# paullric/tempestmodel

Hardware: AMD Instinct MI355X
Metric: element-DOF-updates/s (JW baroclinic wave ne30 np4 L30, ARS343 IMEX) (higher is better)
Workload: dtype f64

## Files before the change

include/tempest_mi355x.h:

```cpp
#ifndef TEMPEST_MI355X_H
#define TEMPEST_MI355X_H

#ifdef __cplusplus
extern "C" {
#endif

#define TMX_ABI_VERSION 5

#define TMX_OK                 0
#define TMX_ERR_INVALID       -1
#define TMX_ERR_UNSUPPORTED   -2
#define TMX_ERR_DEVICE        -3
#define TMX_ERR_SINGULAR      -4
#define TMX_ERR_COMM          -5

typedef struct tmx_engine tmx_engine;

enum {
	TMX_OP_INTERP_NODE_TO_REDGE = 0,
	TMX_OP_INTERP_REDGE_TO_NODE,
	TMX_OP_DIFF_NODE_TO_NODE,
	TMX_OP_DIFF_NODE_TO_REDGE,
	TMX_OP_DIFF_REDGE_TO_NODE,
	TMX_OP_DIFF_REDGE_TO_REDGE,
// ... 185 lines not shown
	TMX_INFO_PHYSICS_KERNEL
};
long long tmx_info(tmx_engine * e, int what);

int tmx_set_option(tmx_engine * e, const char * name, double value);
int tmx_get_option(tmx_engine * e, const char * name, double * value);
typedef void (*tmx_dgbsv_fn)(const int * n, const int * kl, const int * ku, const int * nrhs, double * ab, const int * ldab, int * ipiv,
	double * b, const int * ldb, int * info);
int tmx_lu_flavour_from_dgbsv(tmx_engine * e, tmx_dgbsv_fn dgbsv);
int tmx_options_report(tmx_engine * e, char * buf, int cap);
int tmx_options_from_environment(tmx_engine * e);

int tmx_plan_get(tmx_engine * e, int what, int * out, int cap);
int tmx_plan_get_matrices(tmx_engine * e, double * out, int cap);
int tmx_debug_unique_tables(tmx_engine * e, int tile_shape, int what, int * out, int cap);
int tmx_debug_program_unique(int scheme, int first_step, int last_step);
int tmx_debug_program_mixed(int scheme, int first_step, int last_step, int instance);
int tmx_debug_program_rayleigh(int scheme, int first_step, int last_step);
int tmx_debug_program_prefix(int scheme, int first_step, int last_step, int * pairs, int * terms, int cap);
int tmx_debug_walk_segments(int option, int ntiles, int rows, int target_wavefronts);
int tmx_debug_h_timing(tmx_engine * e, unsigned long long * out);
int tmx_debug_h_walk_timing(tmx_engine * e, unsigned long long * out);

int tmx_debug_dss_loopback(tmx_engine ** engines, int n, int instance);
int tmx_debug_loopback_group(tmx_engine ** engines, int n);
int tmx_debug_comm_selftest(tmx_engine * e);

int tmx_debug_pivot_stats(tmx_engine * e, int enable, unsigned long long out[2]);

int tmx_debug_program_copies(int scheme, int mode, int steps, int share, int * copies, int * shared);
// ... 16 lines not shown
```

tempestmodel_amd/csrc/tmx_device.h:

```cpp
#pragma once
#include "tmx_internal.h"
#include "tmx_refmath.h"

#ifndef TMX_H_FUSE_W
#define TMX_H_FUSE_W 1
#endif
#ifndef KT_H
#define KT_H 4
#endif

#ifdef TMX_LU_NOFMA
#define LU_UPD(a, l, u) ((a) - (l) * (u))
#else
#define LU_UPD(a, l, u) __builtin_fma(-(l), (u), (a))
#endif
#ifndef TMX_STORE_PRED
#define TMX_STORE_PRED true
#endif
#ifndef TMX_TAIL
#define TMX_TAIL 2
#endif
#ifndef TMX_SEARCH_TREE
#define TMX_SEARCH_TREE 0
#endif
// ... 443 lines not shown
#endif
	return (base < 0) ? -1 : base + ((lane >> 2) & 3) * nj + (lane & 3);
}

template <bool UQ> __device__ __forceinline__ bool wg_tile(const KParams & p, int nyb, int & tile_ix, int & yb) {
	if (!UQ) { tile_ix = blockIdx.x; yb = blockIdx.y; return true; }
	if (p.u_xcd) return xcd_tile(p.u_ntiles, nyb, tile_ix, yb);
	tile_ix = blockIdx.x % p.u_ntiles; yb = blockIdx.x / p.u_ntiles;
	return yb < nyb;
}
static inline dim3 wg_grid(bool uq, const KParams & p, int ntiles, int nyb) {
	if (!uq) return dim3(ntiles, nyb);
	return dim3(p.u_xcd ? 8 * ((ntiles + 7) / 8) * nyb : ntiles * nyb);
}

template <int NV, int RL>
__device__ __forceinline__ void seam_store(const KParams & p, double (*srow)[RL], int lane_, int sdst, int sred, const double (&v)[NV],
	double * __restrict__ xo, const int (&slab)[NV], int nv)
{
	const int lane = lds_pos<RL != 64>(lane_);
#ifdef TMX_ABL_UQ_DSTORES
	{
		const int c = min((int)(blockIdx.x & 1023) * 64 + lane, p.NSS - 1);
#pragma unroll
		for (int t = 0; t < NV; t++) if (t < nv) xo[(size_t)slab[t] * p.NSS + c] = v[t];
		return;
	}
#endif
#pragma unroll
	for (int t = 0; t < NV; t++) if (t < nv) srow[t][lane] = v[t];
	__builtin_amdgcn_fence(__ATOMIC_RELEASE, "wavefront");
// ... 8 lines not shown
		const int l1 = lds_pos<RL != 64>((sred >> 4) & 63);
#pragma unroll
		for (int t = 0; t < NV; t++) if (t < nv) o[t] = 0.5 * (v[t] + srow[t][l1]);
	} else if (n == 4) {
		const int l1 = lds_pos<RL != 64>((sred >> 4) & 63), l2 = lds_pos<RL != 64>((sred >> 10) & 63), l3 = lds_pos<RL != 64>((sred >> 16) & 63);
#pragma unroll
		for (int t = 0; t < NV; t++) if (t < nv) {
			const double p0 = v[t] + srow[t][l1], p1 = srow[t][l2] + srow[t][l3];
			o[t] = 0.5 * (0.5 * p0 + 0.5 * p1);
		}
	}
	if (sdst >= 0) {
#pragma unroll
		for (int t = 0; t < NV; t++) if (t < nv) xo[(size_t)slab[t] * p.NSS + sdst] = o[t];
	} else {
		const int q = -2 - sdst;
#pragma unroll
		for (int t = 0; t < NV; t++) if (t < nv) p.part[(size_t)slab[t] * p.NP + q] = o[t];
	}
}

__device__ __forceinline__ void lds_barrier() { asm volatile("s_waitcnt lgkmcnt(0)\n\ts_barrier" ::: "memory"); }
template <int NV>
__device__ __forceinline__ void block_seam_store(const KParams & p, double (*xrow)[256], int pos, int sdst, int sred, const double (&v)[NV],
	double * __restrict__ xo, const int (&slab)[NV], unsigned vmask)
{
#pragma unroll
	for (int t = 0; t < NV; t++) if ((vmask >> t) & 1u) xrow[t][pos] = v[t];
	lds_barrier();
	if (sdst == -1) return;
	const int n = sred & 15;
	double o[NV];
#pragma unroll
	for (int t = 0; t < NV; t++) o[t] = v[t];
	if (n == 2) {
		const int l1 = (sred >> 4) & 255;
#pragma unroll
		for (int t = 0; t < NV; t++) if ((vmask >> t) & 1u) o[t] = 0.5 * (v[t] + xrow[t][l1]);
	} else if (n == 4) {
		const int l1 = (sred >> 4) & 255, l2 = (sred >> 12) & 255, l3 = (sred >> 20) & 255;
#pragma unroll
		for (int t = 0; t < NV; t++) if ((vmask >> t) & 1u) {
			const double p0 = v[t] + xrow[t][l1], p1 = xrow[t][l2] + xrow[t][l3];
			o[t] = 0.5 * (0.5 * p0 + 0.5 * p1);
		}
	}
	if (sdst >= 0) {
#pragma unroll
		for (int t = 0; t < NV; t++) if ((vmask >> t) & 1u) xo[(size_t)slab[t] * p.NSS + sdst] = o[t];
	} else {
		const int q = -2 - sdst;
#pragma unroll
		for (int t = 0; t < NV; t++) if ((vmask >> t) & 1u) p.part[(size_t)slab[t] * p.NP + q] = o[t];
	}
}
```

tempestmodel_amd/csrc/tmx_hostshared.h:

```cpp
#pragma once
#include "tmx_internal.h"
#include <pthread.h>
#include <algorithm>
#include <cmath>
#include <cstdarg>
#include <cstdio>
#include <cstring>
#include <dlfcn.h>
#include <map>
#include <mutex>
#include <numeric>
#include <functional>
#include <thread>

static inline bool plan_only(const tmx_engine * e) { return e->cfg.device == -2; }

typedef struct { char internal[128]; } nccl_uid;
typedef int (*fn_ncclGetUniqueId)(nccl_uid *);
typedef int (*fn_ncclCommInitRank)(void **, int, nccl_uid, int);
typedef int (*fn_ncclCommDestroy)(void *);
typedef int (*fn_ncclGroupStart)(void);
typedef int (*fn_ncclGroupEnd)(void);
typedef int (*fn_ncclSend)(const void *, size_t, int, int, void *, hipStream_t);
typedef int (*fn_ncclRecv)(void *, size_t, int, int, void *, hipStream_t);
// ... 33 lines not shown

template <class T> static int dev_upload(T ** d, const std::vector<T> & h, size_t * bytes) {
	const size_t n = h.size() ? h.size() : 1;
	HIPCHK(hipMalloc((void **)d, n * sizeof(T)));
	if (h.size()) HIPCHK(hipMemcpy(*d, h.data(), h.size() * sizeof(T), hipMemcpyHostToDevice));
	*bytes += n * sizeof(T);
	return TMX_OK;
}

static inline int col_of(const PatchInfo & P, int i, int j) {
	const int a = (i - 1) / TMX_NP, ii = (i - 1) % TMX_NP, b = (j - 1) / TMX_NP, jj = (j - 1) % TMX_NP;
	return (P.elem_base + a * P.neb + b) * TMX_NQ + ii * TMX_NP + jj;
}


static inline size_t p2p_header_bytes(int n_ranks) { return (((size_t)2 * n_ranks * sizeof(unsigned long long)) + 255) / 256 * 256; }

KParams make_params(const tmx_engine * e);
int launch_check(const char * what);
int settle_instance(tmx_engine * e, int ix, bool read_only = false);
int check_ready(tmx_engine * e);
int check_inst(tmx_engine * e, int ix, bool read_only = false);
double * inst(tmx_engine * e, int ix);
void interp_orphan(tmx_engine * e);
const double * inst_uv(tmx_engine * e, int ix);
void drop_readers(tmx_engine * e, int x);
double * uinst(tmx_engine * e, int ix);
const double * uinst_uv(tmx_engine * e, int ix);
int u_own_uv(tmx_engine * e, int ix, bool total = false);
void u_written(tmx_engine * e, int x);
// ... 47 lines not shown
```

tempestmodel_amd/csrc/tmx_k_exchange.hip:

```cpp
#include "tmx_device.h"


#ifndef TMX_DSS_LPT
#define TMX_DSS_LPT 1
#endif
#ifndef TMX_DSS_MINWG
#define TMX_DSS_MINWG 5
#endif
__global__ __launch_bounds__(256, TMX_DSS_MINWG) void k_dss(KParams p, double * __restrict__ x, const double * __restrict__ ghost,
	const int * __restrict__ gbase, const int * __restrict__ gstride, int ngroups, const int * __restrict__ gcols,
	const int * __restrict__ gn, const int * __restrict__ gx, const int * __restrict__ gtype, const double * __restrict__ xmat, int nt, int g0)
{
	const int L = p.L;
	const size_t NS = (size_t)p.NS;
	int bx, by;
	if (!xcd_tile((ngroups - g0 + 63) / 64, (L + 1 + 4 * TMX_DSS_LPT - 1) / (4 * TMX_DSS_LPT), bx, by)) return;
	const int g = g0 + bx * 64 + threadIdx.x;
	const int kk0 = (by * 4 + WAVE_UNIFORM(threadIdx.y)) * TMX_DSS_LPT;
	if (g >= ngroups || kk0 > L) return;
	const int n = gn[g];
	const int4 c4 = *(const int4 *)(gcols + g * 4);
	const int c[4] = { c4.x, c4.y, c4.z, c4.w };
	const int xi = gx[g];
	const int gt = gtype[g];
// ... 62 lines not shown
		}
	}
#undef DSS_SCALAR
	}
}

void tmxk_dss(tmx_engine * e, const KParams & p, double * x, int g0, int g1) {
	if (g1 <= g0) return;
	const int nx = (g1 - g0 + 63) / 64, ny = (p.L + 1 + 4 * TMX_DSS_LPT - 1) / (4 * TMX_DSS_LPT);
	dim3 blk(64, 4), grd(8 * ((nx + 7) / 8) * ny);
	hipLaunchKernelGGL(k_dss, grd, blk, 0, e->stream, p, x, (const double *)e->d_ghost, (const int *)e->d_ghost_base,
		(const int *)e->d_ghost_stride, g1,
		(const int *)e->d_grp_cols, (const int *)e->d_grp_n, (const int *)e->d_grp_x, (const int *)e->d_grp_type, (const double *)e->d_xmat, e->nt, g0);
}

__global__ __launch_bounds__(256) void k_pack(int nslab, size_t NS, int nsend,
	const double * __restrict__ x, const int * __restrict__ cols, const int * __restrict__ base,
	const int * __restrict__ stride, double * __restrict__ buf)
{
	const int i = blockIdx.x * 256 + threadIdx.x;
	const int sl = blockIdx.y;
	if (i >= nsend) return;
	buf[(size_t)base[i] + (size_t)sl * stride[i]] = x[(size_t)sl * NS + cols[i]];
}

void tmxk_pack(tmx_engine * e, const KParams & p, const double * x) {
	if (e->nsend == 0) return;
	dim3 blk(256), grd((e->nsend + 255) / 256, e->nslab);
	hipLaunchKernelGGL(k_pack, grd, blk, 0, e->stream, e->nslab, (size_t)p.NS, e->nsend,
		x, (const int *)e->d_send_cols, (const int *)e->d_send_base, (const int *)e->d_send_stride, e->d_sendbuf);
}

__global__ __launch_bounds__(256) void k_pack_p2p(int nslab, size_t NS, int nsend,
	const double * __restrict__ x, const int * __restrict__ cols, const int * __restrict__ within,
	const int * __restrict__ stride, const int * __restrict__ peer, double * const * __restrict__ dst)
{
	const int i = blockIdx.x * 256 + threadIdx.x;
	const int sl = blockIdx.y;
	if (i >= nsend) return;
	dst[peer[i]][(size_t)sl * stride[i] + within[i]] = x[(size_t)sl * NS + cols[i]];
}

__global__ __launch_bounds__(64) void k_p2p_signal_wait(int npeers, const int * __restrict__ peers, unsigned long long * const * __restrict__ flag_dst,
	const unsigned long long * own, unsigned long long seq, int * __restrict__ fail, unsigned long long timeout_ticks)
{
	for (int q = threadIdx.x; q < npeers; q += 64) {
		__threadfence_system();
		__hip_atomic_store(flag_dst[peers[q]], seq, __ATOMIC_RELEASE, __HIP_MEMORY_SCOPE_SYSTEM);
	}
	const bool failed = (__hip_atomic_load(fail, __ATOMIC_RELAXED, __HIP_MEMORY_SCOPE_AGENT) & TMX_FLAG_COMM) != 0;
	for (int q = threadIdx.x; q < npeers && !failed; q += 64) {
		const unsigned long long t0 = wall_clock64();
		while (__hip_atomic_load(own + peers[q], __ATOMIC_ACQUIRE, __HIP_MEMORY_SCOPE_SYSTEM) < seq) {
			__builtin_amdgcn_s_sleep(8);
			if (timeout_ticks && wall_clock64() - t0 > timeout_ticks) { atomicOr(fail, TMX_FLAG_COMM); break; }
		}
	}
	__threadfence_system();
}

void tmxk_pack_p2p(tmx_engine * e, const KParams & p, const double * x, int buf) {
	if (e->nsend == 0) return;
	dim3 blk(256), grd((e->nsend + 255) / 256, e->nslab);
	hipLaunchKernelGGL(k_pack_p2p, grd, blk, 0, e->stream, e->nslab, (size_t)p.NS, e->nsend,
		x, (const int *)e->d_send_cols, (const int *)e->d_send_within, (const int *)e->d_send_stride, (const int *)e->d_send_peer,
		(double * const *)(e->d_p2p_dst + (size_t)buf * e->cfg.n_ranks));
}

void tmxuk_pack(tmx_engine * e) {
	if (e->nsend == 0) return;
	dim3 blk(256), grd((e->nsend + 255) / 256, e->nslab);
	hipLaunchKernelGGL(k_pack, grd, blk, 0, e->stream, e->nslab, (size_t)e->u.NP, e->nsend,
		(const double *)e->u.d_part, (const int *)e->u.d_send_slots, (const int *)e->d_send_base, (const int *)e->d_send_stride, e->d_sendbuf);
}
void tmxuk_pack_p2p(tmx_engine * e, int buf) {
	if (e->nsend == 0) return;
	dim3 blk(256), grd((e->nsend + 255) / 256, e->nslab);
	hipLaunchKernelGGL(k_pack_p2p, grd, blk, 0, e->stream, e->nslab, (size_t)e->u.NP, e->nsend,
		(const double *)e->u.d_part, (const int *)e->u.d_send_slots, (const int *)e->d_send_within, (const int *)e->d_send_stride, (const int *)e->d_send_peer,
		(double * const *)(e->d_p2p_dst + (size_t)buf * e->cfg.n_ranks));
}

void tmxk_p2p_signal_wait(tmx_engine * e, hipStream_t s, int buf, unsigned long long seq) {
	const unsigned long long timeout_ticks = 100000000ull * (unsigned long long)e->p2p_timeout_s;
	hipLaunchKernelGGL(k_p2p_signal_wait, dim3(1), dim3(64), 0, s, e->p2p_npeers, (const int *)e->d_p2p_peers,
		(unsigned long long * const *)(e->d_p2p_flag + (size_t)buf * e->cfg.n_ranks),
		(const unsigned long long *)e->p2p_block + (size_t)buf * e->cfg.n_ranks, seq, e->d_flag, timeout_ticks);
}



__global__ __launch_bounds__(256) void k_lincomb(size_t n, double * __restrict__ dst, LinTerms t) {
	size_t i = (size_t)blockIdx.x * 256 + threadIdx.x;
	const size_t stride = (size_t)gridDim.x * 256;
	for (; i < n; i += stride) {
// ... 202 lines not shown
```

tempestmodel_amd/csrc/tmx_k_horizontal.hip:

```cpp
#include "tmx_device.h"


#ifdef TMX_H_TIMING
#define HT_WAVES 65536
__device__ unsigned long long g_h_rec[8][HT_WAVES][8];
#define HT_DECL long long ht_ = __builtin_readcyclecounter(); long long hts_[7] = { 0, 0, 0, 0, 0, 0, 0 }
#define HT_MARK(i) do { const long long t1_ = __builtin_readcyclecounter(); hts_[i] += t1_ - ht_; ht_ = t1_; } while (0)
#define HT_END(NT_) do { if (threadIdx.x == 0) { const unsigned w_ = ((blockIdx.x * gridDim.y + blockIdx.y) * KT_H + threadIdx.y) % HT_WAVES; \
	for (int q_ = 0; q_ < 7; q_++) g_h_rec[(NT_) & 7][w_][q_] = (unsigned long long)hts_[q_]; g_h_rec[(NT_) & 7][w_][7] = 1ull; } } while (0)
void tmxk_h_timing_read(unsigned long long * out) {
	static std::vector<unsigned long long> h((size_t)8 * HT_WAVES * 8);
	hipMemcpyFromSymbol(h.data(), HIP_SYMBOL(g_h_rec), h.size() * sizeof(unsigned long long));
	for (int i = 0; i < 128; i++) out[i] = 0;
	for (int nt = 0; nt < 8; nt++) for (int w = 0; w < HT_WAVES; w++) if (h[((size_t)nt * HT_WAVES + w) * 8 + 7])
		for (int q = 0; q < 8; q++) out[nt * 8 + q] += h[((size_t)nt * HT_WAVES + w) * 8 + q];
	std::fill(h.begin(), h.end(), 0ull);
	hipMemcpyToSymbol(HIP_SYMBOL(g_h_rec), h.data(), h.size() * sizeof(unsigned long long));
}
#else
#define HT_DECL
#define HT_MARK(i)
#define HT_END(NT_)
void tmxk_h_timing_read(unsigned long long * out) { for (int i = 0; i < 128; i++) out[i] = 0; }
#endif
// ... 301 lines not shown
		}
		outU = bU + tU; outV = bV + tV;
		if (k < 2) { uv01[(size_t)k * NS + col] = outU; uv01[(size_t)(2 + k) * NS + col] = outV; }
		if (k < L - 1) { outU += tUhi; outV += tVhi; }
		if (k > 0) { outU += tUlo; outV += tVlo; }
		outR = bR - tR; outT = bT - tT;
		if (withW) outW = bW + tW;
		if (!UQ) {
			stu(xup + sU, colb, outU); stu(xup + sV, colb, outV); stu(xup + sR, colb, outR); stu(xup + sT, colb, outT);
			if (withW) stu(xup + TMX_SLAB_W(L, k) * NS, colb, outW);
		}
	}
	if (UQ && !MF) {
		const double v[5] = { outU, outV, outR, outT, outW };
		const int slab[5] = { TMX_SLAB_U(L, k), TMX_SLAB_V(L, k), TMX_SLAB_R(L, k), TMX_SLAB_T(L, k), TMX_SLAB_W(L, k) };
		seam_store<5, TMX_UQ_ROWLEN(UQ)>(p, &s[ty][1], lane, sdst, sred, v, xup, slab, (TMX_H_FUSE_W && ty > 0) ? 5 : 4);
	}
#ifdef TMX_H_TIMING
	asm volatile("s_waitcnt vmcnt(0)" ::: "memory");
#endif
	HT_MARK(6);
	HT_END(NT);
}

template <int NT, bool UQ, bool EM, bool DM = false>
__global__ __launch_bounds__(256) void k_h_w_update(KParams p, LinTerms xbase, double * xup,
	const double * __restrict__ ucz, const double * __restrict__ uv01, double dt, int stride, EmitTerms em)
{
	__shared__ double sw[UQ ? 4 : 1][1][64];
	const int L = p.L;
	const size_t NS = (size_t)p.NS;
// ... 462 lines not shown
	el_stiff(s[ty], sSw[ty], ep, { 0, 2, 4 }, { 1, 3, 5 }, { 6, 7 }, ida, idb, wa, wb, ga, gb);

	const double oW = el_scalar_update(bW, dt, 1.0 / je, nu_s, wa[2], wb[2]);
	double oT = 0, oR = 0, oU = 0, oV = 0;
	if (actn) {
		const double invJ = 1.0 / jn;
		oT = el_scalar_update(bT, dt, invJ, nu_s, wa[0], wb[0]);
		oR = el_scalar_update(bR, dt, invJ, nu_s, wa[1], wb[1]);
		const ElPair up = el_vector_update(nu_d, nu_v, j2d, c2a0, c2a1, c2b1, ga[0], gb[0], ga[1], gb[1]);
		oU = bU - dt * up.a;
		oV = bV - dt * up.b;
	}
	if (UQ) {
		const double v[5] = { oW, oT, oR, oU, oV };
		const int slab[5] = { TMX_SLAB_W(L, kk), TMX_SLAB_T(L, kk), TMX_SLAB_R(L, kk), TMX_SLAB_U(L, kk), TMX_SLAB_V(L, kk) };
		if constexpr (BLK) block_seam_store<5>(p, xs, ty * 64 + lane, sdst, sred, v, xout, slab, (kk < L) ? 31u : 1u);
		else seam_store<5, TMX_UQ_ROWLEN(UQ)>(p, &s[ty][0], lane, sdst, sred, v, xout, slab, (kk < L) ? 5 : 1);
		return;
	}
	xout[TMX_SLAB_W(L, kk) * NS + col] = oW;
	if (actn) {
		xout[TMX_SLAB_T(L, kk) * NS + col] = oT;
		xout[TMX_SLAB_R(L, kk) * NS + col] = oR;
		xout[TMX_SLAB_U(L, kk) * NS + col] = oU;
		xout[TMX_SLAB_V(L, kk) * NS + col] = oV;
	}
}

void tmxk_hypervis(tmx_engine * e, const KParams & p, const double * xsrc, const double * xbase, double * xout,
	double dt, double nu_s, double nu_d, double nu_v, int scale, bool pull_dss) {
	const int ntiles = p.quads ? e->launch_tiles : p.NS / 64, nyb = (p.L + 1 + 3) / 4;
	dim3 blk(64, 4);
// ... 349 lines not shown
```

tempestmodel_amd/csrc/tmx_k_hwalk.hip:

```cpp
#include "tmx_device.h"

#ifdef TMX_H_TIMING
#define HW_WAVES 32768
__device__ unsigned long long g_hw_rec[8][HW_WAVES][8];
#define HW_DECL long long hw_ = __builtin_readcyclecounter(); long long hws_[7] = { 0, 0, 0, 0, 0, 0, 0 }
#define HW_MARK(i) do { const long long t1_ = __builtin_readcyclecounter(); hws_[i] += t1_ - hw_; hw_ = t1_; } while (0)
#define HW_END(NT_) do { if (threadIdx.x == 0) { const unsigned w_ = blockIdx.x % HW_WAVES; \
	for (int q_ = 0; q_ < 7; q_++) g_hw_rec[(NT_) & 7][w_][q_] = (unsigned long long)hws_[q_]; g_hw_rec[(NT_) & 7][w_][7] = 1ull; } } while (0)
void tmxk_h_walk_timing_read(unsigned long long * out) {
	static std::vector<unsigned long long> h((size_t)8 * HW_WAVES * 8);
	hipMemcpyFromSymbol(h.data(), HIP_SYMBOL(g_hw_rec), h.size() * sizeof(unsigned long long));
	for (int i = 0; i < 128; i++) out[i] = 0;
	for (int nt = 0; nt < 8; nt++) for (int w = 0; w < HW_WAVES; w++) if (h[((size_t)nt * HW_WAVES + w) * 8 + 7])
		for (int q = 0; q < 8; q++) out[nt * 8 + q] += h[((size_t)nt * HW_WAVES + w) * 8 + q];
	std::fill(h.begin(), h.end(), 0ull);
	hipMemcpyToSymbol(HIP_SYMBOL(g_hw_rec), h.data(), h.size() * sizeof(unsigned long long));
}
#else
#define HW_DECL
#define HW_MARK(i)
#define HW_END(NT_)
void tmxk_h_walk_timing_read(unsigned long long * out) { for (int i = 0; i < 128; i++) out[i] = 0; }
#endif

// ... 410 lines not shown
				double ub0 = 0.0, vb0 = 0.0;
				ub0 += OPK(TMX_OP_INTERP_NODE_TO_REDGE, 0, 0) * uh0; ub0 += OPK(TMX_OP_INTERP_NODE_TO_REDGE, 0, 1) * uh;
				vb0 += OPK(TMX_OP_INTERP_NODE_TO_REDGE, 0, 0) * vh0; vb0 += OPK(TMX_OP_INTERP_NODE_TO_REDGE, 0, 1) * vh;
				double e0, e1, e2, ea, eb_;
				met_eval(mc, etac[L], e0, e1, e2, ea, eb_);
				extra = -(e0 * ub0 + e1 * vb0) / e2; vmask |= 32u;
			}
			if (k == L - 1) {
				double xWl[NX];
				terms_load<NT, PM, DM>(xbase.src, dmask, TMX_SLAB_W(L, L), SS, NSD, cb, gd, xWl);
				extra = lin_reduce<NT, PM>(xbase, xWl); xslab = TMX_SLAB_W(L, L); vmask |= 32u;
				if (EM) stu(em.xp + TMX_SLAB_W(L, L) * SS, cb, emit_value<NT>(em, xWl));
			}
			const double v[6] = { outU, outV, outR, outT, outW, extra };
			const int slab[6] = { TMX_SLAB_U(L, k), TMX_SLAB_V(L, k), TMX_SLAB_R(L, k), TMX_SLAB_T(L, k), TMX_SLAB_W(L, k), xslab };
			block_seam_store<6>(p, xs[k & 1], pos, sdst, sred, v, xup, slab, vmask);
		} else {
			{
				const double v[5] = { outU, outV, outR, outT, outW };
				const int slab[5] = { TMX_SLAB_U(L, k), TMX_SLAB_V(L, k), TMX_SLAB_R(L, k), TMX_SLAB_T(L, k), TMX_SLAB_W(L, k) };
				seam_store<5, RL>(p, &s[0], lane, sdst, sred, v, xup, slab, (k > 0) ? 5 : 4);
			}
			if (k == 0) { uh0 = uh; vh0 = vh; }
			if (k == 1) {
				wave_sync();
				double ub0 = 0.0, vb0 = 0.0;
				ub0 += OPK(TMX_OP_INTERP_NODE_TO_REDGE, 0, 0) * uh0; ub0 += OPK(TMX_OP_INTERP_NODE_TO_REDGE, 0, 1) * uh;
				vb0 += OPK(TMX_OP_INTERP_NODE_TO_REDGE, 0, 0) * vh0; vb0 += OPK(TMX_OP_INTERP_NODE_TO_REDGE, 0, 1) * vh;
				double e0, e1, e2, ea, eb_;
				met_eval(mc, etac[L], e0, e1, e2, ea, eb_);
				const double v1[1] = { -(e0 * ub0 + e1 * vb0) / e2 };
				const int slab1[1] = { TMX_SLAB_W(L, 0) };
				seam_store<1, RL>(p, &s[0], lane, sdst, sred, v1, xup, slab1, 1);
			}
		}
		wave_sync();
// ... 230 lines not shown
		if (actn) {
			oT = c.bT - dt * invJ * nu_s * (uaT + ubT);
			oR = c.bR - dt * invJ * nu_s * (uaR + ubR);
			const double upa = nu_d * dad - nu_v * j2d * (c2a1 * dac + c2b1 * dbc);
			const double upb = nu_d * dbd + nu_v * j2d * (c2a0 * dac + c2a1 * dbc);
			oU = c.bU - dt * upa;
			oV = c.bV - dt * upb;
		}
		wave_sync();
		c = nx;
		asm volatile("" : "+v"(c.W), "+v"(c.T), "+v"(c.R), "+v"(c.U), "+v"(c.V));
		if (HB) asm volatile("" : "+v"(c.bW), "+v"(c.bT), "+v"(c.bR), "+v"(c.bU), "+v"(c.bV));
		{
			const double v[5] = { oW, oT, oR, oU, oV };
			const int slab[5] = { TMX_SLAB_W(L, kk), TMX_SLAB_T(L, kk), TMX_SLAB_R(L, kk), TMX_SLAB_U(L, kk), TMX_SLAB_V(L, kk) };
			seam_store<5, RL>(p, &s[0], lane, here ? sdst : -1, sred, v, xout, slab, actn ? 5 : 1);
		}
		wave_sync();
	};
	Lev C, N;
	load_level(C, k0);
	wave_sync();
	for (int kl = k0; kl < k1; kl++) {
		const int kk = WAVE_UNIFORM(kl);
		level(kk, C, N, N, min(kk + 1, k1 - 1));
	}
}

bool tmxk_hv_walk_ok(const tmx_engine * e, const KParams & p) { return p.t_ucol != nullptr && e->opt_hv_walk != 0 && !tmxu_blocks_on(e, 2); }

void tmxk_hv_walk(tmx_engine * e, const KParams & p, const double * xsrc, const double * xbase, double * xout, double dt, double nu_s, double nu_d, double nu_v, int scale) {
// ... 11 lines not shown
```

tempestmodel_amd/csrc/tmx_plan.hip:

```cpp
#include "tmx_hostshared.h"


struct NodeRef { int patch, i, j; };

struct Nodes {
	const tmx_engine * e;
	std::vector<size_t> poff;
	explicit Nodes(const tmx_engine * e_) : e(e_), poff(e_->cfg.n_patches + 1, 0) {
		for (int p = 0; p < e->cfg.n_patches; p++) poff[p + 1] = poff[p] + (size_t)e->patches[p].na * e->patches[p].nb;
	}
	int id(int p, int i, int j) const { return (int)(poff[p] + (size_t)i * e->patches[p].nb + j); }
	NodeRef ref(int id) const {
		const int p = (int)(std::upper_bound(poff.begin(), poff.end(), (size_t)id) - poff.begin()) - 1;
		const int loc = id - (int)poff[p];
		return NodeRef{ p, loc / e->patches[p].nb, loc % e->patches[p].nb };
	}
	bool local(int id) const { return e->patches[ref(id).patch].owner == e->cfg.rank; }
	int col(int id) const { const NodeRef nr = ref(id); return col_of(e->patches[nr.patch], nr.i, nr.j); }
};
typedef std::vector<std::vector<int>> Groups;

static int uf_find(std::vector<int> & par, int x) {
	while (par[x] != x) { par[x] = par[par[x]]; x = par[x]; }
	return x;
// ... 401 lines not shown
		for (const std::vector<int> * t : { &plan.send_base, &plan.send_stride, &plan.ghost_base, &plan.ghost_stride }) v.insert(v.end(), t->begin(), t->end());
	} else if (what == 10) {
		v = plan.send_cols;
	} else return -1;
	if (out) { if ((int)v.size() > cap) return -1; if (!v.empty()) memcpy(out, v.data(), v.size() * sizeof(int)); }
	return (int)v.size();
}

extern "C" int tmx_plan_get_matrices(tmx_engine * e, double * out, int cap) {
	if (!e || !e->finalized) return -1;
	const PlanHost & plan = e->plan;
	if (out) { if ((int)plan.xmat.size() > cap) return -1; if (!plan.xmat.empty()) memcpy(out, plan.xmat.data(), plan.xmat.size() * sizeof(double)); }
	return (int)plan.xmat.size();
}

extern "C" int tmx_debug_unique_tables(tmx_engine * e, int tile_shape, int what, int * out, int cap) {
	if (!e || !e->finalized || tile_shape < 0 || tile_shape > 4) return -1;
	UniqueLayout keep = e->u;
	e->u = UniqueLayout(); e->u.tile_shape = tile_shape;
	UniqueTables T;
	const int r = tmxu_tables(e, T);
	const UniqueLayout u = e->u;
	e->u = keep;
	if (r) return -1;
	std::vector<int> v;
	switch (what) {
		case 0: v = { u.NU, u.NUS, u.NTS, u.nslots, u.ngroups, u.ngroups_local, u.n_early, u.n_late, u.b_ngroups, u.b_ngroups_local, u.nblocks, u.nb_early, u.nb_late }; break;
		case 13: v = T.b_sdst; break; case 14: v = T.b_sred; break; case 15: v = T.blk_info; break; case 16: v = T.b_gsrc; break; case 17: v = T.b_gdst; break; case 18: v = T.b_gn; break;
		case 19: v = T.blks_early; break; case 20: v = T.blks_late; break;
		case 1: v = T.t_dcol; break; case 2: v = T.t_ucol; break; case 3: v = T.t_sdst; break; case 4: v = T.t_sred; break;
// ... 8 lines not shown
```

tempestmodel_amd/csrc/tmx_unique.hip:

```cpp
#include "tmx_device.h"
#include "tmx_hostshared.h"
#include <algorithm>
#include <cstring>
#include <map>

static int floor_half(int v) { return (v >= 0) ? v / 2 : -((-v + 1) / 2); }
static int sign_of(int v) { return (v > 0) - (v < 0); }
static void gilbert_rec(int x, int y, int ax, int ay, int bx, int by, std::vector<std::pair<int, int>> & out) {
	const int w = std::abs(ax + ay), h = std::abs(bx + by);
	const int dax = sign_of(ax), day = sign_of(ay), dbx = sign_of(bx), dby = sign_of(by);
	if (h == 1) { for (int q = 0; q < w; q++) { out.push_back({ x, y }); x += dax; y += day; } return; }
	if (w == 1) { for (int q = 0; q < h; q++) { out.push_back({ x, y }); x += dbx; y += dby; } return; }
	int ax2 = floor_half(ax), ay2 = floor_half(ay), bx2 = floor_half(bx), by2 = floor_half(by);
	const int w2 = std::abs(ax2 + ay2), h2 = std::abs(bx2 + by2);
	if (2 * w > 3 * h) {
		if ((w2 % 2) && w > 2) { ax2 += dax; ay2 += day; }
		gilbert_rec(x, y, ax2, ay2, bx, by, out);
		gilbert_rec(x + ax2, y + ay2, ax - ax2, ay - ay2, bx, by, out);
	} else {
		if ((h2 % 2) && h > 2) { bx2 += dbx; by2 += dby; }
		gilbert_rec(x, y, bx2, by2, ax2, ay2, out);
		gilbert_rec(x + bx2, y + by2, ax, ay, bx - bx2, by - by2, out);
		gilbert_rec(x + (ax - dax) + (bx2 - dbx), y + (ay - day) + (by2 - dby), -bx2, -by2, -(ax - ax2), -(ay - ay2), out);
	}
// ... 366 lines not shown
	if (u.form[slot] == 2) {
		if (!keep_u) { u.form[slot] = 0; u.n_uform--; }
		return TMX_OK;
	}
	double * xd = e->d_state + (size_t)slot * e->inst_stride;
	const double * xu = u.d_ustate + (size_t)u.uslot[slot] * u.ustride;
	const int ny = std::min(e->nslab, 64);
	hipLaunchKernelGGL(k_u_to_d, dim3((e->ncol + 255) / 256, ny), dim3(256), 0, e->stream, e->nslab, (size_t)e->NS, (size_t)u.NUS, e->ncol, xu, xd, (const int *)u.d_ucol_of_dcol);
	u.conversions++;
	if (keep_u) u.form[slot] = 2;
	else { u.form[slot] = 0; u.n_uform--; }
	return TMX_OK;
}


__global__ __launch_bounds__(256) void k_slots_from_u(int nslab, size_t NUS, size_t NP, int nslots, const double * __restrict__ xu, double * __restrict__ part,
	const int * __restrict__ slot_ucol)
{
	const int q = blockIdx.x * 256 + threadIdx.x;
	if (q >= nslots) return;
	const int uu = slot_ucol[q];
	for (int s = blockIdx.y; s < nslab; s += gridDim.y) part[(size_t)s * NP + q] = xu[(size_t)s * NUS + uu];
}

void tmxuk_slots_from_u(tmx_engine * e, const double * xu) {
	const UniqueLayout & u = e->u;
	if (u.nslots == 0) return;
	hipLaunchKernelGGL(k_slots_from_u, dim3((u.nslots + 255) / 256, std::min(e->nslab, 64)), dim3(256), 0, e->stream, e->nslab, (size_t)u.NUS, (size_t)u.NP, u.nslots, xu,
		u.d_part, (const int *)u.d_slot_ucol);
}

template <int vc>
__device__ __forceinline__ void dss_u_body(int L, size_t NUS, size_t NP, double * __restrict__ xu, const double * __restrict__ part,
	const double * __restrict__ ghost, const int * __restrict__ gbase, const int * __restrict__ gstride, int ngroups, const int * __restrict__ gsrc,
	const int * __restrict__ gdst, const int * __restrict__ gn, const int * __restrict__ gx, const int * __restrict__ gtype, const double * __restrict__ xmat, int g, int kk)
{
	if (vc > 0 && kk >= L) return;
	const int n = gn[g];
	const int4 c4 = *(const int4 *)(gsrc + g * 4), d4 = *(const int4 *)(gdst + g * 4);
	const int c[4] = { c4.x, c4.y, c4.z, c4.w }, d[4] = { d4.x, d4.y, d4.z, d4.w };
	const int xi = gx[g], gt = gtype[g];
	const double * ptr[4]; size_t str[4];
#pragma unroll
	for (int m = 0; m < 4; m++) {
		if (m >= n) { ptr[m] = part; str[m] = 0; }
		else if (c[m] < (int)NP) { ptr[m] = part + c[m]; str[m] = NP; }
		else { ptr[m] = ghost + gbase[c[m] - (int)NP]; str[m] = (size_t)gstride[c[m] - (int)NP]; }
	}
	const bool lev = (kk < L);
	int slabs[5];
	slabs[0] = TMX_SLAB_W(L, kk);
	slabs[1] = lev ? TMX_SLAB_T(L, kk) : slabs[0]; slabs[2] = lev ? TMX_SLAB_R(L, kk) : slabs[0];
	slabs[3] = lev ? TMX_SLAB_U(L, kk) : slabs[0]; slabs[4] = lev ? TMX_SLAB_V(L, kk) : slabs[0];
	auto mine = [&](int t) { return vc == 3 ? t >= 3 : t == vc; };
	double v[5][4];
#pragma unroll
	for (int t = 0; t < 5; t++)
#pragma unroll
		for (int m = 0; m < 4; m++) v[t][m] = (m < n && (t == 0 || lev) && mine(t)) ? ptr[m][(size_t)slabs[t] * str[m]] : 0.0;
	const bool same = (gt == 0) && (n != 3);
	const int t0 = gt & 3, t1 = (gt >> 2) & 3, t2 = (gt >> 4) & 3, t3 = (gt >> 6) & 3;
#define DSS_SCALAR(W0, W1, W2, W3, O0, O1, O2, O3) do { \
		if (same) { const double a_ = dss_combine<0>(W0, W1, W2, W3, n, 0); O0 = a_; O1 = a_; O2 = a_; O3 = a_; } \
		else { O0 = dss_combine<0>(W0, W1, W2, W3, n, t0); O1 = dss_combine<1>(W0, W1, W2, W3, n, t1); \
		       O2 = dss_combine<2>(W0, W1, W2, W3, n, t2); O3 = dss_combine<3>(W0, W1, W2, W3, n, t3); } } while (0)
	double out[5][4];
#pragma unroll
	for (int t = 0; t < 3; t++) if (mine(t)) DSS_SCALAR(v[t][0], v[t][1], v[t][2], v[t][3], out[t][0], out[t][1], out[t][2], out[t][3]);
	if (!mine(3)) { }
	else if (xi < 0) {
		DSS_SCALAR(v[3][0], v[3][1], v[3][2], v[3][3], out[3][0], out[3][1], out[3][2], out[3][3]);
		DSS_SCALAR(v[4][0], v[4][1], v[4][2], v[4][3], out[4][0], out[4][1], out[4][2], out[4][3]);
	} else {
		const double * Mx = xmat + (size_t)xi * 64;
// ... 1 lines not shown
			A_ = T_[0] * v[3][Q_] + T_[1] * v[4][Q_]; B_ = T_[2] * v[3][Q_] + T_[3] * v[4][Q_]; } } while (0)
#define DSS_VEC(M_, TY_) do { double a0, a1, a2, a3, b0, b1, b2, b3; \
			DSS_ROT(M_, 0, a0, b0); DSS_ROT(M_, 1, a1, b1); DSS_ROT(M_, 2, a2, b2); DSS_ROT(M_, 3, a3, b3); \
			out[3][M_] = dss_combine<M_>(a0, a1, a2, a3, n, TY_); out[4][M_] = dss_combine<M_>(b0, b1, b2, b3, n, TY_); } while (0)
		DSS_VEC(0, t0); DSS_VEC(1, t1); DSS_VEC(2, t2); DSS_VEC(3, t3);
#undef DSS_VEC
#undef DSS_ROT
	}
#pragma unroll
	for (int t = 0; t < 5; t++)
#pragma unroll
		for (int m = 0; m < 4; m++)
			if (d[m] >= 0 && (t == 0 || lev) && mine(t)) xu[(size_t)slabs[t] * NUS + d[m]] = out[t][m];
#undef DSS_SCALAR
}
__global__ __launch_bounds__(256, 8) void k_dss_u(int L, int nt, size_t NUS, size_t NP, double * __restrict__ xu, const double * __restrict__ part,
	const double * __restrict__ ghost, const int * __restrict__ gbase, const int * __restrict__ gstride, int ngroups, const int * __restrict__ gsrc,
	const int * __restrict__ gdst, const int * __restrict__ gn, const int * __restrict__ gx, const int * __restrict__ gtype, const double * __restrict__ xmat, int g0)
{
	int bx, by;
	(void)nt;
	if (!xcd_tile((ngroups - g0 + 63) / 64, L + 1, bx, by)) return;
	const int kk = by, vc = WAVE_UNIFORM(threadIdx.y);
	const int g = g0 + bx * 64 + threadIdx.x;
	if (g >= ngroups || kk > L) return;
#define DSS_GO(VC_) dss_u_body<VC_>(L, NUS, NP, xu, part, ghost, gbase, gstride, ngroups, gsrc, gdst, gn, gx, gtype, xmat, g, kk)
	if (vc == 0) DSS_GO(0); else if (vc == 1) DSS_GO(1); else if (vc == 2) DSS_GO(2); else DSS_GO(3);
#undef DSS_GO
}

void tmxuk_dss(tmx_engine * e, double * xu, int g0, int g1, bool blocks) {
	if (g1 <= g0) return;
	const UniqueLayout & u = e->u;
	const int nx = (g1 - g0 + 63) / 64, ny = e->L + 1;
	hipLaunchKernelGGL(k_dss_u, dim3(8 * ((nx + 7) / 8) * ny), dim3(64, 4), 0, e->stream, e->L, e->nt, (size_t)u.NUS, (size_t)u.NP, xu, (const double *)u.d_part,
		(const double *)e->d_ghost, (const int *)e->d_ghost_base, (const int *)e->d_ghost_stride, g1, (const int *)(blocks ? u.d_b_gsrc : u.d_gsrc), (const int *)(blocks ? u.d_b_gdst : u.d_gdst),
		(const int *)(blocks ? u.d_b_gn : u.d_gn), (const int *)(blocks ? u.d_b_gx : u.d_gx), (const int *)(blocks ? u.d_b_gtype : u.d_gtype), (const double *)e->d_xmat, g0);
}


void tmxuk_gather_rows(tmx_engine * e, int nrows, const double * xd, double * xu) {
	const UniqueLayout & u = e->u;
	hipLaunchKernelGGL(k_d_to_u, dim3((u.NU + 255) / 256, std::min(nrows, 64)), dim3(256), 0, e->stream, nrows, (size_t)e->NS, (size_t)u.NUS, u.NU, xd, xu, (const int *)u.d_u_rep);
}

int tmxu_physics_inputs(tmx_engine * e, bool * ok) {
	UniqueLayout & u = e->u;
	if (u.physics_dirty) {
		static_assert(G2_PS == G2_LAT + 1 && G2_SINLAT == G2_LAT + 2 && G2_COSLAT == G2_LAT + 3, "physics input rows are contiguous");
		const double * xd = e->d_g2d + (size_t)G2_LAT * e->NS;
// ... 14 lines not shown
```

Baseline: 11.49 billion.

## Interleave paired slabs in seam partial buffer and pair DSS wave loads

Changes the layout of the seam partial buffer so that U/V slabs and R/T slabs are interleaved per node, letting seam stores write double2 pairs and DSS kernels read both components with one 16-byte load. The DSS kernel is regrouped from four waves (W, T, R, UV) to three (W, TR, UV), with the block size and launch bounds adjusted to match. Pack and slots-from-u kernels are updated to address the new layout, and a debug offset helper is added. This trades simpler indexing for fewer, wider memory transactions, at the cost of less parallelism in DSS and more complex address arithmetic.

New measurement: 11.51 billion (median of 2 runs). Within noise of the previous version (+0.1%).

```diff
diff --git a/include/tempest_mi355x.h b/include/tempest_mi355x.h
--- a/include/tempest_mi355x.h
+++ b/include/tempest_mi355x.h
@@ -223,6 +223,7 @@
 int tmx_plan_get(tmx_engine * e, int what, int * out, int cap);
 int tmx_plan_get_matrices(tmx_engine * e, double * out, int cap);
 int tmx_debug_unique_tables(tmx_engine * e, int tile_shape, int what, int * out, int cap);
+long long tmx_debug_unique_offset(int L, int N, int slab, int node);
 int tmx_debug_program_unique(int scheme, int first_step, int last_step);
 int tmx_debug_program_mixed(int scheme, int first_step, int last_step, int instance);
 int tmx_debug_program_rayleigh(int scheme, int first_step, int last_step);
diff --git a/tempestmodel_amd/csrc/tmx_device.h b/tempestmodel_amd/csrc/tmx_device.h
--- a/tempestmodel_amd/csrc/tmx_device.h
+++ b/tempestmodel_amd/csrc/tmx_device.h
@@ -481,7 +481,36 @@
 	return dim3(p.u_xcd ? 8 * ((ntiles + 7) / 8) * nyb : ntiles * nyb);
 }
 
-template <int NV, int RL>
+struct PairOff { size_t row; unsigned lane; };
+__device__ __forceinline__ size_t pair_row(int L, size_t N, int slab0) { return (size_t)(2 * slab0 - ((slab0 >= 2 * L) ? 2 * L : 0)) * N; }
+__device__ __forceinline__ PairOff pair_off(int L, size_t N, int slab, int node) {
+	if (slab >= 4 * L) return { (size_t)slab * N, (unsigned)node * 8u };
+	const int rb = (slab >= 2 * L) ? 2 * L : 0, comp = (slab - rb >= L) ? 1 : 0;
+	return { (size_t)(rb + 2 * (slab - rb - comp * L)) * N, (unsigned)node * 16u + (unsigned)comp * 8u };
+}
+__device__ __forceinline__ void st_pair(double * uniform_base, unsigned lane_byte_off, double a, double b) {
+	*(double2 *)((char *)uniform_base + lane_byte_off) = make_double2(a, b);
+}
+enum { SO_NONE = 0, SO_UVRTW = 1, SO_WTRUV = 2 };
+template <int ORD, int NV, class ON>
+__device__ __forceinline__ void slot_store(const KParams & p, int q, const double (&o)[NV], const int (&slab)[NV], ON on) {
+	asm volatile("" : "+v"(q));
+	static_assert(ORD == SO_NONE || NV >= 5, "a paired order names five values");
+	constexpr bool PR = ORD != SO_NONE;
+	constexpr int a0 = !PR ? 0 : ((ORD == SO_UVRTW) ? 0 : 3), b0 = !PR ? 0 : ((ORD == SO_UVRTW) ? 1 : 4);
+	constexpr int a1 = !PR ? 0 : ((ORD == SO_UVRTW) ? 3 : 1), b1 = !PR ? 0 : 2;
+	const size_t NP = (size_t)p.NP;
+#pragma unroll
+	for (int t = 0; t < NV; t++) {
+		if (!on(t)) continue;
+		if (PR && (t == b0 || t == b1)) continue;
+		if (PR && t == a0) st_pair(p.part + (size_t)(2 * slab[a0]) * NP, (unsigned)q * 16u, o[a0], o[b0]);
+		else if (PR && t == a1) st_pair(p.part + (size_t)(2 * slab[a1] - 2 * p.L) * NP, (unsigned)q * 16u, o[a1], o[b1]);
+		else if (PR) stu(p.part + (size_t)slab[t] * NP, (unsigned)q * 8u, o[t]);
+		else { const PairOff w = pair_off(p.L, NP, slab[t], q); stu(p.part + w.row, w.lane, o[t]); }
+	}
+}
+template <int NV, int RL, int ORD = SO_NONE>
 __device__ __forceinline__ void seam_store(const KParams & p, double (*srow)[RL], int lane_, int sdst, int sred, const double (&v)[NV],
 	double * __restrict__ xo, const int (&slab)[NV], int nv)
 {
@@ -520,14 +549,12 @@
 #pragma unroll
 		for (int t = 0; t < NV; t++) if (t < nv) xo[(size_t)slab[t] * p.NSS + sdst] = o[t];
 	} else {
-		const int q = -2 - sdst;
-#pragma unroll
-		for (int t = 0; t < NV; t++) if (t < nv) p.part[(size_t)slab[t] * p.NP + q] = o[t];
+		slot_store<ORD>(p, -2 - sdst, o, slab, [&](int t) { return t < nv; });
 	}
 }
 
 __device__ __forceinline__ void lds_barrier() { asm volatile("s_waitcnt lgkmcnt(0)\n\ts_barrier" ::: "memory"); }
-template <int NV>
+template <int NV, int ORD = SO_NONE>
 __device__ __forceinline__ void block_seam_store(const KParams & p, double (*xrow)[256], int pos, int sdst, int sred, const double (&v)[NV],
 	double * __restrict__ xo, const int (&slab)[NV], unsigned vmask)
 {
@@ -555,8 +582,6 @@
 #pragma unroll
 		for (int t = 0; t < NV; t++) if ((vmask >> t) & 1u) xo[(size_t)slab[t] * p.NSS + sdst] = o[t];
 	} else {
-		const int q = -2 - sdst;
-#pragma unroll
-		for (int t = 0; t < NV; t++) if ((vmask >> t) & 1u) p.part[(size_t)slab[t] * p.NP + q] = o[t];
-	}
-}
+		slot_store<ORD>(p, -2 - sdst, o, slab, [&](int t) { return ((vmask >> t) & 1u) != 0u; });
+	}
+}
diff --git a/tempestmodel_amd/csrc/tmx_hostshared.h b/tempestmodel_amd/csrc/tmx_hostshared.h
--- a/tempestmodel_amd/csrc/tmx_hostshared.h
+++ b/tempestmodel_amd/csrc/tmx_hostshared.h
@@ -71,6 +71,12 @@
 }
 
 
+static inline size_t pair_offset_host(int L, size_t N, int slab, int node) {
+	if (slab >= 4 * L) return (size_t)slab * N + (size_t)node;
+	const int rb = (slab >= 2 * L) ? 2 * L : 0, comp = (slab - rb >= L) ? 1 : 0;
+	return (size_t)(rb + 2 * (slab - rb - comp * L)) * N + (size_t)node * 2 + (size_t)comp;
+}
+
 static inline size_t p2p_header_bytes(int n_ranks) { return (((size_t)2 * n_ranks * sizeof(unsigned long long)) + 255) / 256 * 256; }
 
 KParams make_params(const tmx_engine * e);
diff --git a/tempestmodel_amd/csrc/tmx_k_exchange.hip b/tempestmodel_amd/csrc/tmx_k_exchange.hip
--- a/tempestmodel_amd/csrc/tmx_k_exchange.hip
+++ b/tempestmodel_amd/csrc/tmx_k_exchange.hip
@@ -100,31 +100,36 @@
 		(const int *)e->d_grp_cols, (const int *)e->d_grp_n, (const int *)e->d_grp_x, (const int *)e->d_grp_type, (const double *)e->d_xmat, e->nt, g0);
 }
 
+__device__ __forceinline__ double pack_source(const double * __restrict__ x, int pairL, size_t NS, int sl, int col) {
+	if (!pairL) return x[(size_t)sl * NS + col];
+	const PairOff w = pair_off(pairL, NS, sl, col);
+	return ldu(x + w.row, w.lane);
+}
 __global__ __launch_bounds__(256) void k_pack(int nslab, size_t NS, int nsend,
 	const double * __restrict__ x, const int * __restrict__ cols, const int * __restrict__ base,
-	const int * __restrict__ stride, double * __restrict__ buf)
+	const int * __restrict__ stride, double * __restrict__ buf, int pairL)
 {
 	const int i = blockIdx.x * 256 + threadIdx.x;
 	const int sl = blockIdx.y;
 	if (i >= nsend) return;
-	buf[(size_t)base[i] + (size_t)sl * stride[i]] = x[(size_t)sl * NS + cols[i]];
+	buf[(size_t)base[i] + (size_t)sl * stride[i]] = pack_source(x, pairL, NS, sl, cols[i]);
 }
 
 void tmxk_pack(tmx_engine * e, const KParams & p, const double * x) {
 	if (e->nsend == 0) return;
 	dim3 blk(256), grd((e->nsend + 255) / 256, e->nslab);
 	hipLaunchKernelGGL(k_pack, grd, blk, 0, e->stream, e->nslab, (size_t)p.NS, e->nsend,
-		x, (const int *)e->d_send_cols, (const int *)e->d_send_base, (const int *)e->d_send_stride, e->d_sendbuf);
+		x, (const int *)e->d_send_cols, (const int *)e->d_send_base, (const int *)e->d_send_stride, e->d_sendbuf, 0);
 }
 
 __global__ __launch_bounds__(256) void k_pack_p2p(int nslab, size_t NS, int nsend,
 	const double * __restrict__ x, const int * __restrict__ cols, const int * __restrict__ within,
-	const int * __restrict__ stride, const int * __restrict__ peer, double * const * __restrict__ dst)
+	const int * __restrict__ stride, const int * __restrict__ peer, double * const * __restrict__ dst, int pairL)
 {
 	const int i = blockIdx.x * 256 + threadIdx.x;
 	const int sl = blockIdx.y;
 	if (i >= nsend) return;
-	dst[peer[i]][(size_t)sl * stride[i] + within[i]] = x[(size_t)sl * NS + cols[i]];
+	dst[peer[i]][(size_t)sl * stride[i] + within[i]] = pack_source(x, pairL, NS, sl, cols[i]);
 }
 
 __global__ __launch_bounds__(64) void k_p2p_signal_wait(int npeers, const int * __restrict__ peers, unsigned long long * const * __restrict__ flag_dst,
@@ -150,21 +155,21 @@
 	dim3 blk(256), grd((e->nsend + 255) / 256, e->nslab);
 	hipLaunchKernelGGL(k_pack_p2p, grd, blk, 0, e->stream, e->nslab, (size_t)p.NS, e->nsend,
 		x, (const int *)e->d_send_cols, (const int *)e->d_send_within, (const int *)e->d_send_stride, (const int *)e->d_send_peer,
-		(double * const *)(e->d_p2p_dst + (size_t)buf * e->cfg.n_ranks));
+		(double * const *)(e->d_p2p_dst + (size_t)buf * e->cfg.n_ranks), 0);
 }
 
 void tmxuk_pack(tmx_engine * e) {
 	if (e->nsend == 0) return;
 	dim3 blk(256), grd((e->nsend + 255) / 256, e->nslab);
 	hipLaunchKernelGGL(k_pack, grd, blk, 0, e->stream, e->nslab, (size_t)e->u.NP, e->nsend,
-		(const double *)e->u.d_part, (const int *)e->u.d_send_slots, (const int *)e->d_send_base, (const int *)e->d_send_stride, e->d_sendbuf);
+		(const double *)e->u.d_part, (const int *)e->u.d_send_slots, (const int *)e->d_send_base, (const int *)e->d_send_stride, e->d_sendbuf, e->L);
 }
 void tmxuk_pack_p2p(tmx_engine * e, int buf) {
 	if (e->nsend == 0) return;
 	dim3 blk(256), grd((e->nsend + 255) / 256, e->nslab);
 	hipLaunchKernelGGL(k_pack_p2p, grd, blk, 0, e->stream, e->nslab, (size_t)e->u.NP, e->nsend,
 		(const double *)e->u.d_part, (const int *)e->u.d_send_slots, (const int *)e->d_send_within, (const int *)e->d_send_stride, (const int *)e->d_send_peer,
-		(double * const *)(e->d_p2p_dst + (size_t)buf * e->cfg.n_ranks));
+		(double * const *)(e->d_p2p_dst + (size_t)buf * e->cfg.n_ranks), e->L);
 }
 
 void tmxk_p2p_signal_wait(tmx_engine * e, hipStream_t s, int buf, unsigned long long seq) {
diff --git a/tempestmodel_amd/csrc/tmx_k_horizontal.hip b/tempestmodel_amd/csrc/tmx_k_horizontal.hip
--- a/tempestmodel_amd/csrc/tmx_k_horizontal.hip
+++ b/tempestmodel_amd/csrc/tmx_k_horizontal.hip
@@ -339,7 +339,7 @@
 	if (UQ && !MF) {
 		const double v[5] = { outU, outV, outR, outT, outW };
 		const int slab[5] = { TMX_SLAB_U(L, k), TMX_SLAB_V(L, k), TMX_SLAB_R(L, k), TMX_SLAB_T(L, k), TMX_SLAB_W(L, k) };
-		seam_store<5, TMX_UQ_ROWLEN(UQ)>(p, &s[ty][1], lane, sdst, sred, v, xup, slab, (TMX_H_FUSE_W && ty > 0) ? 5 : 4);
+		seam_store<5, TMX_UQ_ROWLEN(UQ), SO_UVRTW>(p, &s[ty][1], lane, sdst, sred, v, xup, slab, (TMX_H_FUSE_W && ty > 0) ? 5 : 4);
 	}
 #ifdef TMX_H_TIMING
 	asm volatile("s_waitcnt vmcnt(0)" ::: "memory");
@@ -832,8 +832,8 @@
 	if (UQ) {
 		const double v[5] = { oW, oT, oR, oU, oV };
 		const int slab[5] = { TMX_SLAB_W(L, kk), TMX_SLAB_T(L, kk), TMX_SLAB_R(L, kk), TMX_SLAB_U(L, kk), TMX_SLAB_V(L, kk) };
-		if constexpr (BLK) block_seam_store<5>(p, xs, ty * 64 + lane, sdst, sred, v, xout, slab, (kk < L) ? 31u : 1u);
-		else seam_store<5, TMX_UQ_ROWLEN(UQ)>(p, &s[ty][0], lane, sdst, sred, v, xout, slab, (kk < L) ? 5 : 1);
+		if constexpr (BLK) block_seam_store<5, SO_WTRUV>(p, xs, ty * 64 + lane, sdst, sred, v, xout, slab, (kk < L) ? 31u : 1u);
+		else seam_store<5, TMX_UQ_ROWLEN(UQ), SO_WTRUV>(p, &s[ty][0], lane, sdst, sred, v, xout, slab, (kk < L) ? 5 : 1);
 		return;
 	}
 	xout[TMX_SLAB_W(L, kk) * NS + col] = oW;
diff --git a/tempestmodel_amd/csrc/tmx_k_hwalk.hip b/tempestmodel_amd/csrc/tmx_k_hwalk.hip
--- a/tempestmodel_amd/csrc/tmx_k_hwalk.hip
+++ b/tempestmodel_amd/csrc/tmx_k_hwalk.hip
@@ -448,12 +448,12 @@
 			}
 			const double v[6] = { outU, outV, outR, outT, outW, extra };
 			const int slab[6] = { TMX_SLAB_U(L, k), TMX_SLAB_V(L, k), TMX_SLAB_R(L, k), TMX_SLAB_T(L, k), TMX_SLAB_W(L, k), xslab };
-			block_seam_store<6>(p, xs[k & 1], pos, sdst, sred, v, xup, slab, vmask);
+			block_seam_store<6, SO_UVRTW>(p, xs[k & 1], pos, sdst, sred, v, xup, slab, vmask);
 		} else {
 			{
 				const double v[5] = { outU, outV, outR, outT, outW };
 				const int slab[5] = { TMX_SLAB_U(L, k), TMX_SLAB_V(L, k), TMX_SLAB_R(L, k), TMX_SLAB_T(L, k), TMX_SLAB_W(L, k) };
-				seam_store<5, RL>(p, &s[0], lane, sdst, sred, v, xup, slab, (k > 0) ? 5 : 4);
+				seam_store<5, RL, SO_UVRTW>(p, &s[0], lane, sdst, sred, v, xup, slab, (k > 0) ? 5 : 4);
 			}
 			if (k == 0) { uh0 = uh; vh0 = vh; }
 			if (k == 1) {
@@ -714,7 +714,7 @@
 		{
 			const double v[5] = { oW, oT, oR, oU, oV };
 			const int slab[5] = { TMX_SLAB_W(L, kk), TMX_SLAB_T(L, kk), TMX_SLAB_R(L, kk), TMX_SLAB_U(L, kk), TMX_SLAB_V(L, kk) };
-			seam_store<5, RL>(p, &s[0], lane, here ? sdst : -1, sred, v, xout, slab, actn ? 5 : 1);
+			seam_store<5, RL, SO_WTRUV>(p, &s[0], lane, here ? sdst : -1, sred, v, xout, slab, actn ? 5 : 1);
 		}
 		wave_sync();
 	};
diff --git a/tempestmodel_amd/csrc/tmx_plan.hip b/tempestmodel_amd/csrc/tmx_plan.hip
--- a/tempestmodel_amd/csrc/tmx_plan.hip
+++ b/tempestmodel_amd/csrc/tmx_plan.hip
@@ -439,6 +439,11 @@
 	return (int)plan.xmat.size();
 }
 
+extern "C" long long tmx_debug_unique_offset(int L, int N, int slab, int node) {
+	if (L < 1 || N < 1 || slab < 0 || slab > 5 * L || node < 0 || node >= N) return -1;
+	return (long long)pair_offset_host(L, (size_t)N, slab, node);
+}
+
 extern "C" int tmx_debug_unique_tables(tmx_engine * e, int tile_shape, int what, int * out, int cap) {
 	if (!e || !e->finalized || tile_shape < 0 || tile_shape > 4) return -1;
 	UniqueLayout keep = e->u;
diff --git a/tempestmodel_amd/csrc/tmx_unique.hip b/tempestmodel_amd/csrc/tmx_unique.hip
--- a/tempestmodel_amd/csrc/tmx_unique.hip
+++ b/tempestmodel_amd/csrc/tmx_unique.hip
@@ -404,19 +404,22 @@
 }
 
 
-__global__ __launch_bounds__(256) void k_slots_from_u(int nslab, size_t NUS, size_t NP, int nslots, const double * __restrict__ xu, double * __restrict__ part,
+__global__ __launch_bounds__(256) void k_slots_from_u(int L, int nslab, size_t NUS, size_t NP, int nslots, const double * __restrict__ xu, double * __restrict__ part,
 	const int * __restrict__ slot_ucol)
 {
 	const int q = blockIdx.x * 256 + threadIdx.x;
 	if (q >= nslots) return;
 	const int uu = slot_ucol[q];
-	for (int s = blockIdx.y; s < nslab; s += gridDim.y) part[(size_t)s * NP + q] = xu[(size_t)s * NUS + uu];
+	for (int s = blockIdx.y; s < nslab; s += gridDim.y) {
+		const PairOff w = pair_off(L, NP, s, q);
+		stu(part + w.row, w.lane, xu[(size_t)s * NUS + uu]);
+	}
 }
 
 void tmxuk_slots_from_u(tmx_engine * e, const double * xu) {
 	const UniqueLayout & u = e->u;
 	if (u.nslots == 0) return;
-	hipLaunchKernelGGL(k_slots_from_u, dim3((u.nslots + 255) / 256, std::min(e->nslab, 64)), dim3(256), 0, e->stream, e->nslab, (size_t)u.NUS, (size_t)u.NP, u.nslots, xu,
+	hipLaunchKernelGGL(k_slots_from_u, dim3((u.nslots + 255) / 256, std::min(e->nslab, 64)), dim3(256), 0, e->stream, e->L, e->nslab, (size_t)u.NUS, (size_t)u.NP, u.nslots, xu,
 		u.d_part, (const int *)u.d_slot_ucol);
 }
 
@@ -430,24 +433,31 @@
 	const int4 c4 = *(const int4 *)(gsrc + g * 4), d4 = *(const int4 *)(gdst + g * 4);
 	const int c[4] = { c4.x, c4.y, c4.z, c4.w }, d[4] = { d4.x, d4.y, d4.z, d4.w };
 	const int xi = gx[g], gt = gtype[g];
-	const double * ptr[4]; size_t str[4];
-#pragma unroll
-	for (int m = 0; m < 4; m++) {
-		if (m >= n) { ptr[m] = part; str[m] = 0; }
-		else if (c[m] < (int)NP) { ptr[m] = part + c[m]; str[m] = NP; }
-		else { ptr[m] = ghost + gbase[c[m] - (int)NP]; str[m] = (size_t)gstride[c[m] - (int)NP]; }
-	}
 	const bool lev = (kk < L);
 	int slabs[5];
 	slabs[0] = TMX_SLAB_W(L, kk);
 	slabs[1] = lev ? TMX_SLAB_T(L, kk) : slabs[0]; slabs[2] = lev ? TMX_SLAB_R(L, kk) : slabs[0];
 	slabs[3] = lev ? TMX_SLAB_U(L, kk) : slabs[0]; slabs[4] = lev ? TMX_SLAB_V(L, kk) : slabs[0];
-	auto mine = [&](int t) { return vc == 3 ? t >= 3 : t == vc; };
+	auto mine = [&](int t) { return vc == 0 ? t == 0 : (vc == 1 ? (t == 1 || t == 2) : t >= 3); };
+	constexpr int ta = (vc == 0) ? 0 : ((vc == 1) ? 1 : 3), tb = (vc == 0) ? 0 : ta + 1;
 	double v[5][4];
 #pragma unroll
 	for (int t = 0; t < 5; t++)
 #pragma unroll
-		for (int m = 0; m < 4; m++) v[t][m] = (m < n && (t == 0 || lev) && mine(t)) ? ptr[m][(size_t)slabs[t] * str[m]] : 0.0;
+		for (int m = 0; m < 4; m++) v[t][m] = 0.0;
+	const size_t prow = (vc == 0) ? (size_t)slabs[0] * NP : pair_row(L, NP, slabs[ta]);
+#pragma unroll
+	for (int m = 0; m < 4; m++) {
+		if (m >= n) continue;
+		if (c[m] < (int)NP) {
+			if (vc == 0) v[0][m] = part[prow + c[m]];
+			else { const double2 w = *(const double2 *)(part + prow + 2 * (size_t)c[m]); v[ta][m] = w.x; v[tb][m] = w.y; }
+		} else {
+			const double * gp = ghost + gbase[c[m] - (int)NP]; const size_t gs = (size_t)gstride[c[m] - (int)NP];
+			v[ta][m] = gp[(size_t)slabs[ta] * gs];
+			if (vc != 0) v[tb][m] = gp[(size_t)slabs[tb] * gs];
+		}
+	}
 	const bool same = (gt == 0) && (n != 3);
 	const int t0 = gt & 3, t1 = (gt >> 2) & 3, t2 = (gt >> 4) & 3, t3 = (gt >> 6) & 3;
 #define DSS_SCALAR(W0, W1, W2, W3, O0, O1, O2, O3) do { \
@@ -479,7 +489,7 @@
 			if (d[m] >= 0 && (t == 0 || lev) && mine(t)) xu[(size_t)slabs[t] * NUS + d[m]] = out[t][m];
 #undef DSS_SCALAR
 }
-__global__ __launch_bounds__(256, 8) void k_dss_u(int L, int nt, size_t NUS, size_t NP, double * __restrict__ xu, const double * __restrict__ part,
+__global__ __launch_bounds__(192, 8) void k_dss_u(int L, int nt, size_t NUS, size_t NP, double * __restrict__ xu, const double * __restrict__ part,
 	const double * __restrict__ ghost, const int * __restrict__ gbase, const int * __restrict__ gstride, int ngroups, const int * __restrict__ gsrc,
 	const int * __restrict__ gdst, const int * __restrict__ gn, const int * __restrict__ gx, const int * __restrict__ gtype, const double * __restrict__ xmat, int g0)
 {
@@ -490,7 +500,7 @@
 	const int g = g0 + bx * 64 + threadIdx.x;
 	if (g >= ngroups || kk > L) return;
 #define DSS_GO(VC_) dss_u_body<VC_>(L, NUS, NP, xu, part, ghost, gbase, gstride, ngroups, gsrc, gdst, gn, gx, gtype, xmat, g, kk)
-	if (vc == 0) DSS_GO(0); else if (vc == 1) DSS_GO(1); else if (vc == 2) DSS_GO(2); else DSS_GO(3);
+	if (vc == 0) DSS_GO(0); else if (vc == 1) DSS_GO(1); else DSS_GO(2);
 #undef DSS_GO
 }
 
@@ -498,7 +508,7 @@
 	if (g1 <= g0) return;
 	const UniqueLayout & u = e->u;
 	const int nx = (g1 - g0 + 63) / 64, ny = e->L + 1;
-	hipLaunchKernelGGL(k_dss_u, dim3(8 * ((nx + 7) / 8) * ny), dim3(64, 4), 0, e->stream, e->L, e->nt, (size_t)u.NUS, (size_t)u.NP, xu, (const double *)u.d_part,
+	hipLaunchKernelGGL(k_dss_u, dim3(8 * ((nx + 7) / 8) * ny), dim3(64, 3), 0, e->stream, e->L, e->nt, (size_t)u.NUS, (size_t)u.NP, xu, (const double *)u.d_part,
 		(const double *)e->d_ghost, (const int *)e->d_ghost_base, (const int *)e->d_ghost_stride, g1, (const int *)(blocks ? u.d_b_gsrc : u.d_gsrc), (const int *)(blocks ? u.d_b_gdst : u.d_gdst),
 		(const int *)(blocks ? u.d_b_gn : u.d_gn), (const int *)(blocks ? u.d_b_gx : u.d_gx), (const int *)(blocks ? u.d_b_gtype : u.d_gtype), (const double *)e->d_xmat, g0);
 }
```
